# sbelharbi/sr-caco-2

Hardware: AMD Instinct MI355X
Metric: train patches/sec, SwinIR x8 64->512 1ch (higher is better)
Workload: dtype f32 (fp16x2 split-MFMA, f32 accumulate)

## Files before the change

### include/srhip.h

```cpp
#ifndef SRHIP_H
#define SRHIP_H
#ifdef __cplusplus
extern "C" {
#endif
#if defined(__GNUC__) || defined(__clang__)
#pragma GCC visibility push(default)
#endif

const char* srhip_last_error(void);
int srhip_abi_version(void);
int srhip_experiments_enabled(void);
int srhip_set_matmul_mode(int mode);
int srhip_get_matmul_mode(void);


int srhip_gemm_nt(const float* A, long lda, const float* W, long ldw, const float* bias, float* C,
                  long ldc, int M, int N, int K, int a_mode, const float* ln_stats, int epi,
                  const float* R, long ldr, const float* rowscale, int rows_per_scale, float alpha,
                  float* aux, long ldaux, void* stream);

int srhip_gemm_nt_batched(const float* A, long lda, long a_z0, long a_z1, const float* W, long ldw, long w_z0, long w_z1, float* C,
                          long ldc, long c_z0, long c_z1, int M, int N, int K, int zcount, int zdiv, void* stream);

int srhip_conv3x3_nhwc(const float* X, long ldx, const float* Wp, const float* bias, float* Y, long ldy,
// ... 13 lines not shown
int srhip_prep_table(const srhip_prep_entry* table_dev, int n, int total_blocks, void* stream);
int srhip_gemm_nt_bx3(const float* A, long lda, const void* Wb, const float* bias, float* C,
                      long ldc, int M, int N, int K, int a_mode, const float* ln_stats, int epi,
                      const float* R, long ldr, const float* rowscale, int rows_per_scale, float alpha,
                      float* aux, long ldaux, float* stats_out, void* stream);
int srhip_gemm_nt_bx3_lnbwd(const float* A, long lda, const void* Wb, float* out, long ldo, int M, int N, int K,
                            const float* x, long ldx, const float* stats, const float* res, long ldres,
                            void* stream);
int srhip_gemm_nt_f16x2(const float* A, long lda, const void* Wh, const float* bias, float* C,
                        long ldc, int M, int N, int K, int a_mode, const float* ln_stats, int epi,
                        const float* R, long ldr, const float* rowscale, int rows_per_scale, float alpha,
                        float* aux, long ldaux, float* stats_out, void* stream);
int srhip_gemm_nt_f16x2_lnbwd(const float* A, long lda, const void* Wh, float* out, long ldo, int M, int N, int K,
                              const float* x, long ldx, const float* stats, const float* res, long ldres,
                              void* stream);
int srhip_conv3x3_nhwc_f16x2(const float* X, long ldx, const void* Wh, const float* bias, float* Y, long ldy,
                             int B, int H, int W, int Cin, int Cout, int epi, const float* R, long ldr,
                             const float* rowscale, float alpha, void* stream);
int srhip_conv3x3_nhwc_split_ex(int wfmt, const float* X, long ldx, const void* Wp, const float* bias, float* Y, long ldy,
                                int B, int H, int W, int Cin, int Cout, int epi, const float* R, long ldr,
                                const float* rowscale, float alpha, const float* in_bn_coef, const float* slope,
                                void* stream);
int srhip_resblock64_fwd_f16x2(const float* x, long ldx, const void* W1h, const float* b1, const void* W2h, const float* b2,
                               float res_scale, float* a, long lda, float* out, long ldout, int B, int H, int W, void* stream);
int srhip_resblock64_bwd_f16x2(const float* g, long ldg, const void* W2Th, const void* W1Th, const float* a, long lda,
                               float res_scale, float* da, long ldda, float* dx, long lddx, int B, int H, int W, void* stream);

int srhip_conv3x3_nhwc_h16(const void* X, long ldx, const void* Wh, const float* bias, void* Y, long ldy, int B, int H, int W,
                           int Cin, int Cout, int epi, const void* R, long ldr, float alpha, int ps2, const float* in_bn_coef,
                           int center_only, void* stream);
// ... 207 lines not shown
int srhip_avgpool2d(const float* x, float* out, int B, int H, int W, int C, int k, void* stream);
int srhip_cpb_bias(const float* table, const long long* index, float* biasT, int heads, int N1, int N2, int entries, void* stream);
int srhip_cosine_window_attention(const float* q, long ldq, int qH, int qW, int qwh, int qww, const float* k, long ldk,
                                  const float* v, long ldv, int kH, int kW, int kwh, int kww, const float* logit_scale,
                                  const float* biasT, float* out, long ldo, int B, int heads, int d, int shift, void* stream);

int srhip_bias_expand_f16x2(const float* table, float* biasF, float* biasG, int heads, void* stream);
int srhip_window_attention_fwd_f16x2(const float* qkv, float* out, const float* biasF, int B, int H, int W, int C,
                                     int heads, int shift, void* stream);
long srhip_window_attention_bwd_f16x2_ws(int B, int H, int W, int heads);
int srhip_window_attention_bwd_f16x2(const float* qkv, const float* dout, float* dqkv, const float* biasF,
                                     const float* biasG, float* dbiasT, float* workspace, int B, int H, int W, int C,
                                     int heads, int shift, void* stream);
int srhip_window_attention_dbias_reduce_f16x2(const float* workspace, long ws_stride, int nblocks, float* dbiasT,
                                              long img_stride, int B, int H, int W, int heads, void* stream);

int srhip_bias_expand(const float* table, float* biasT, float* biasN, int heads, void* stream);
int srhip_bias_grad(const float* dbiasT, float* dtable, int heads, void* stream);
int srhip_bias_grad_batched(const float* dbiasT, long image_stride, float* const* dtables, int nblocks, int heads,
                            void* stream);
int srhip_window_attention_fwd(const float* qkv, float* out, const float* biasT, int B, int H, int W,
                               int C, int heads, int shift, void* stream);
long srhip_window_attention_bwd_ws(int B, int H, int W, int heads);
int srhip_window_attention_bwd(const float* qkv, const float* dout, float* dqkv, const float* biasT,
                               const float* biasN, float* dbiasT, float* workspace, int B, int H, int W,
                               int C, int heads, int shift, void* stream);

int srhip_conv3x3_cin1_fwd(const float* x, const float* w, const float* bias, float* y, long ldy, int B,
                           int H, int W, int Co, int flip, void* stream);
long srhip_conv3x3_cin1_wgrad_ws(int Co);
// ... 189 lines not shown
```

### sr-caco-2_amd/csrc/api.hip

```cpp
#include <stdarg.h>
#include "common.h"
#include "kernels.h"
#include "../../include/srhip.h"

static thread_local char g_err[512] = "";

int sr_fail(int code, const char* fmt, ...) {
  va_list ap;
  va_start(ap, fmt);
  vsnprintf(g_err, sizeof(g_err), fmt, ap);
  va_end(ap);
  return code;
}

extern "C" {

const char* srhip_last_error(void) { return g_err; }
int srhip_abi_version(void) { return 14; }
int srhip_experiments_enabled(void) {
#ifdef SRHIP_EXPERIMENTS
  return 1;
#else
  return 0;
#endif
// ... 93 lines not shown
                      const float* R, long ldr, const float* rowscale, int rows_per_scale, float alpha, float* aux,
                      long ldaux, float* stats_out, void* stream) {
  return gemm_nt_split(0, A, lda, Wb, bias, C, ldc, M, N, K, a_mode, ln_stats, epi, R, ldr, rowscale, rows_per_scale, alpha,
                       aux, ldaux, stats_out, stream);
}
int srhip_gemm_nt_f16x2(const float* A, long lda, const void* Wh, const float* bias, float* C,
                        long ldc, int M, int N, int K, int a_mode, const float* ln_stats, int epi,
                        const float* R, long ldr, const float* rowscale, int rows_per_scale, float alpha, float* aux,
                        long ldaux, float* stats_out, void* stream) {
  return gemm_nt_split(1, A, lda, Wh, bias, C, ldc, M, N, K, a_mode, ln_stats, epi, R, ldr, rowscale, rows_per_scale, alpha,
                       aux, ldaux, stats_out, stream);
}

static int gemm_nt_split_lnbwd(int wfmt, const float* A, long lda, const void* Wb, float* out, long ldo, int M, int N, int K,
                            const float* x, long ldx, const float* stats, const float* res, long ldres,
                            void* stream) {
  NtArgs p;
  memset(&p, 0, sizeof(p));
  p.A = A; p.lda = lda; p.Wb = (const unsigned short*)Wb; p.C = out; p.ldc = ldo;
  p.M = M; p.N = N; p.K = K; p.R = x; p.ldr = ldx; p.R2 = res; p.ldr2 = ldres; p.ep_stats = stats;
  p.alpha = 1.f;
  p.wfmt = wfmt;
  SR_REQUIRE(!wfmt || N % 180 == 0 || N > 128, "gemm_nt_f16x2_lnbwd: N = %d does not run on 192-column tiles", N);
  return sr_gemm_ntb_lnbwd(p, (hipStream_t)stream);
}
int srhip_gemm_nt_bx3_lnbwd(const float* A, long lda, const void* Wb, float* out, long ldo, int M, int N, int K,
                            const float* x, long ldx, const float* stats, const float* res, long ldres,
                            void* stream) {
  return gemm_nt_split_lnbwd(0, A, lda, Wb, out, ldo, M, N, K, x, ldx, stats, res, ldres, stream);
}
int srhip_gemm_nt_f16x2_lnbwd(const float* A, long lda, const void* Wh, float* out, long ldo, int M, int N, int K,
                              const float* x, long ldx, const float* stats, const float* res, long ldres,
                              void* stream) {
  return gemm_nt_split_lnbwd(1, A, lda, Wh, out, ldo, M, N, K, x, ldx, stats, res, ldres, stream);
}

int srhip_mlp_fwd_f16x2(const float* x, long ldx, const float* stats, const void* W1h, const float* b1,
                        const void* W2h, const float* b2, float* h, long ldh, float* out, long ldo, int M, int C,
                        int hidden, const float* rowscale, int rows_per_scale, float* stats_out, void* stream) {
  SR_REQUIRE(x && stats && W1h && b1 && W2h && out, "mlp_fwd_f16x2: null operand");
  SR_REQUIRE(!rowscale || rows_per_scale > 0, "mlp_fwd_f16x2: rows_per_scale must be > 0");
  MlpF16Args p;
  memset(&p, 0, sizeof(p));
  p.X = x; p.ldx = ldx; p.ln_stats = stats;
  p.W1 = (const unsigned short*)W1h; p.N1 = hidden; p.K1 = C; p.Kp1 = sr_kp(C);
  p.W2 = (const unsigned short*)W2h; p.N2 = C; p.K2 = hidden; p.Kp2 = sr_kp(hidden);
  p.b1 = b1; p.b2 = b2; p.H = h; p.ldh = h ? ldh : 4; p.out = out; p.ldo = ldo; p.R = x; p.ldr = ldx;
  p.rowscale = rowscale; p.rows_per_scale = rows_per_scale; p.stats_out = stats_out;
  p.M = M; p.C = C; p.hid = hidden;
// ... 373 lines not shown
```

### sr-caco-2_amd/csrc/kernels.h

```cpp
#pragma once
#include <hip/hip_runtime.h>

struct NtArgs {
  const float* A; long lda;
  const float* W; long ldw; long wtap;
  float* C; long ldc;
  int M, N, K;
  int n_tile;
  int xcd_order;
  const float* bias;
  int a_mode;
  const float* ln_stats;
  int epi;
  const float* slope;
  const float* pro_coef;
  const float* R; long ldr;
  float* aux; long ldaux;
  const float* R2; long ldr2; const float* ep_stats;
  int wide_epi;
  float* stats_out;
  const float* rowscale; int rows_per_scale; float alpha;
  int batch, H, Wd, tiles_x, tiles_y;
  int dbg;
  int stagger;
  const unsigned short* Wb; int Kp;
  int amp;
  int ps;
  int k_rot;
  int wfmt;
  int zcount, zdiv;
  long zA[2], zW[2], zC[2];
};

// ... 132 lines not shown
```

### sr-caco-2_amd/csrc/nt_epi.h

```cpp
#pragma once
#include "common.h"
#include "kernels.h"

__device__ __forceinline__ float half_reduce16(float (&a)[16], int lane) {
#pragma unroll
  for (int n = 8, m = 16; n >= 1; n >>= 1, m >>= 1) {
    const bool up = lane & m;
#pragma unroll
    for (int i = 0; i < n; ++i) {
      const float s = up ? a[i] : a[i + n], k = up ? a[i + n] : a[i];
      a[i] = k + __shfl_xor(s, m, 64);
    }
  }
  return a[0] + __shfl_xor(a[0], 1, 64);
}
__device__ __forceinline__ int half_reduce16_row(int lane) {
  return ((lane >> 4) & 1) * 8 + ((lane >> 3) & 1) * 4 + ((lane >> 2) & 1) * 2 + ((lane >> 1) & 1);
}

template <int WN>
__device__ __forceinline__ void nt_row_stats(const NtArgs& p, f32x16 (&acc)[1][WN], int lane, int wm, int wn,
                                             int m0, int nvalid, float* red) {
  const int r = lane & 31;
  const float inv = 1.0f / (float)p.N;
// ... 229 lines not shown
  }
  const float t1 = half_reduce16(a1, lane), t2 = half_reduce16(a2, lane);
  const int qs = half_reduce16_row(lane);
  __syncthreads();
  if (!(lane & 1)) *(float2*)(red + ((wn * 64) + wm * 32 + mfma_row(qs, lane)) * 2) = float2{t1, t2};
  float rres[WN][16];
#pragma unroll
  for (int j = 0; j < WN; ++j) {
    const int col = min((wn * WN + j) * 32 + r, nvalid - 1);
#pragma unroll
    for (int q = 0; q < 16; ++q) {
      const int g = min(rbase + mfma_row(q, lane), p.M - 1);
      rres[j][q] = p.R2 ? p.R2[(long)g * p.ldr2 + col] : 0.f;
    }
  }
  __syncthreads();
  const float inv = 1.0f / (float)p.N;
#pragma unroll
  for (int q = 0; q < 16; ++q) {
    const int lr = wm * 32 + mfma_row(q, lane);
    const float2 p0 = *(const float2*)(red + lr * 2), p1 = *(const float2*)(red + (64 + lr) * 2);
    const float m1 = (p0.x + p1.x) * inv, m2 = (p0.y + p1.y) * inv;
    const bool rok = rbase + mfma_row(q, lane) < p.M;
#pragma unroll
    for (int j = 0; j < WN; ++j) {
      const int col = (wn * WN + j) * 32 + r;
      if (rok && col < nvalid)
        p.C[(long)(rbase + mfma_row(q, lane)) * p.ldc + col] =
            rres[j][q] + rs[q] * (acc[0][j][q] - m1 - xh[j][q] * m2);
    }
  }
}

template <int WN, bool STATS>
__device__ __forceinline__ void nt_epilogue_wide_impl(const NtArgs& p, f32x16 (&acc)[1][WN], int lane, int wave,
                                                 int wm, int wn, int n0, int nvalid, int m0, float* lds) {
  constexpr int P = 32 * WN + 8;
  constexpr int F4 = 8 * WN;
  constexpr int NIT = 32 * F4 / 64;
  const int r = lane & 31;
  float* tile = lds + wave * (32 * P);
  __syncthreads();
#pragma unroll
  for (int j = 0; j < WN; ++j) {
// ... 112 lines not shown
```

### sr-caco-2_amd/csrc/wattn2.hip

```cpp
#include "common.h"
#include "kernels.h"
#include "wattn2_dev.h"

namespace {

template <int D>
__global__ void __launch_bounds__(256, 3) k_wattn2_fwd(const float* __restrict__ qkv, float* __restrict__ out,
                                                      const float* __restrict__ biasF, long total, int H, int W,
                                                      int C, int heads, int shift, float scale) {
  const int lane = threadIdx.x & 63, wv = threadIdx.x >> 6;
  const long gid = sr_xcd_block(blockIdx.x, gridDim.x) * 4L + wv;
  if (gid >= total) return;
  const W2Geom geo = w2_decode(gid, heads, W / 8, H / 8, shift);
  w2_fwd_body<D>(qkv, out, biasF, geo, H, W, C, shift, scale, lane);
}

template <int D>
__device__ __forceinline__ void w2_gather_cols(const float* __restrict__ base, long pitch, const W2Geom& geo, int H, int W,
                                               int shift, int c, int g, u32x4 (&hi)[2][2], u32x4 (&lo)[2][2],
                                               float (&rinv)[2]) {
  float raw[2][2][8];
#pragma unroll
  for (int JJ = 0; JJ < 2; ++JJ)
#pragma unroll
// ... 27 lines not shown
__device__ __forceinline__ void w2_pack_pair(const f32x4& t0, const f32x4& t1, float sc, u32x4& hi, u32x4& lo) {
  unsigned h[4], l[4];
  split2_pair(t0[0] * sc, t0[1] * sc, h[0], l[0]);
  split2_pair(t0[2] * sc, t0[3] * sc, h[1], l[1]);
  split2_pair(t1[0] * sc, t1[1] * sc, h[2], l[2]);
  split2_pair(t1[2] * sc, t1[3] * sc, h[3], l[3]);
  hi = u32x4{h[0], h[1], h[2], h[3]};
  lo = u32x4{l[0], l[1], l[2], l[3]};
}
__device__ __forceinline__ f32x4 mfma3(const u32x4& ah, const u32x4& al, const u32x4& bh, const u32x4& bl, f32x4 acc) {
  acc = mfma16h(ah, bl, acc);
  acc = mfma16h(al, bh, acc);
  return mfma16h(ah, bh, acc);
}

constexpr int W2_DS = 4096;
constexpr int W3_PL = 64 * 64;
constexpr int W3_IMG = 2 * W3_PL;
constexpr int W3_WPB = 4;
constexpr int W3_LDS = 4 * W3_IMG + (W2_DS + 256 + 4 * 64 + 2 * 64) * 4;

typedef short w3_s16x4 __attribute__((__vector_size__(4 * sizeof(short))));
template <int CTRL>
__device__ __forceinline__ float w3_dpp(float v) {
  return __builtin_bit_cast(float, __builtin_amdgcn_update_dpp(0, __builtin_bit_cast(int, v), CTRL, 0xf, 0xf, true));
}
__device__ __forceinline__ int w3_slot(int row, int u) { return (row * 4 + (u ^ ((row >> 2) & 3))) * 16; }
__device__ __forceinline__ void w3_rows(const unsigned char* img, int T, int c, int g, u32x4& hi, u32x4& lo) {
  const unsigned char* p = img + w3_slot(16 * T + c, g);
  hi = *(const u32x4*)p;
// ... 17 lines not shown
  lo = w3_cols1(img + W3_PL, JJ, jd, c, g);
}
#ifndef W3_OCC
#define W3_OCC 3
#endif
#ifdef SRHIP_EXPERIMENTS
__device__ long long* g_w3_dbg = nullptr;
__device__ int g_w3_mode = 0;
#define W3_MODE(B) (g_w3_mode & (B))
#define SR_TS(K) \
  if (g_w3_dbg && lane == 0) g_w3_dbg[(((long)blockIdx.x * 4 + wv) * W3_WPB + wi) * 8 + (K)] = (long long)wall_clock64();
#else
#define SR_TS(K)
#define W3_MODE(B) 0
#endif
template <int D>
__global__ void __launch_bounds__(256, W3_OCC) k_wattn3_bwd(const float* __restrict__ qkv, const float* __restrict__ dout,
                                                      float* __restrict__ dqkv, const float* __restrict__ biasF,
                                                      float* __restrict__ part,
                                                      int nwin, int H, int W, int C, int heads, int shift, float scale) {
  extern __shared__ __attribute__((aligned(16))) unsigned char w3s[];
  unsigned char* const imQ = w3s;
  unsigned char* const imK = w3s + W3_IMG;
  unsigned char* const imV = w3s + 2 * W3_IMG;
  unsigned char* const imG = w3s + 3 * W3_IMG;
  float* const dsl = (float*)(w3s + 4 * W3_IMG);
  float* const tab = dsl + W2_DS;
  float* const rs = tab + 256;
  float* const lse = rs + 256;
  float* const dlt = lse + 64;
  const int tid = threadIdx.x, lane = tid & 63, c = lane & 15, g = lane >> 4;
  const int wv = __builtin_amdgcn_readfirstlane(tid >> 6);
  const int lb = sr_xcd_block(blockIdx.x, gridDim.x);
  const int head = lb % heads, wg = lb / heads;
// ... 221 lines not shown
          OK[jd] = mfma3(th, tl, dh, dlo, OK[jd]);
        }
      }
      float* op = dqb + (long)w2_token(geo, 16 * J + c, H, W, shift) * C3 + 4 * g;
      if (!W3_MODE(2))
#pragma unroll
      for (int jd = 0; jd < 2; ++jd) {
        w3_store<D>(op + C + 16 * jd, 16 * jd + 4 * g, OK[jd], dri);
        w3_store<D>(op + 2 * C + 16 * jd, 16 * jd + 4 * g, OV[jd], pri);
      }
    }
    SR_TS(5)
    sr_lds_barrier();
    SR_TS(6)
  }
  if (part) {
    float* dst = part + ((long)wg * heads + head) * W2_DS;
#pragma unroll
    for (int J = 0; J < 4; ++J) {
      const int o = w2_img_index(wv, J, lane);
      *(f32x4*)(dst + o) = *(const f32x4*)(dsl + o);
    }
  }
}

__global__ void __launch_bounds__(256) k_dbias2_reduce(const float* __restrict__ part, int nparts, int heads,
                                                       float* __restrict__ dimg, long part_stride, long img_stride) {
  __shared__ double sm[4][64][4];
  const int ln = threadIdx.x & 63, pg = threadIdx.x >> 6;
  const int hd = blockIdx.x >> 4, a = (blockIdx.x >> 3) & 1, b = (blockIdx.x >> 2) & 1, qh = blockIdx.x & 3;
  part += (long)blockIdx.y * part_stride;
  dimg += (long)blockIdx.y * img_stride;
  const int key = mfma_row(4 * qh, ln) + 32 * a, query = (ln & 31) + 32 * b;
  const int mine = w2_img_index(query >> 4, key >> 4, 16 * ((key >> 2) & 3) + (query & 15));
  const float* p = part + (long)hd * W2_DS + mine;
  const long ps = (long)heads * W2_DS;
  double s0 = 0.0, s1 = 0.0, s2 = 0.0, s3 = 0.0;
  int i = pg;
// ... 80 lines not shown
}

int srhip_window_attention_bwd_f16x2(const float* qkv, const float* dout, float* dqkv, const float* biasF,
                                     const float* biasG, float* dbiasT, float* workspace, int B, int H, int W, int C,
                                     int heads, int shift, void* stream) {
  if (int rc = w2_check(B, H, W, C, heads, shift)) return rc;
  SR_REQUIRE(!dbiasT || workspace, "window_attention_bwd_f16x2: workspace required for the bias gradient");
  const int D = C / heads;
  const int nwin = B * (H / 8) * (W / 8), nparts = sr_cdiv(nwin, 4);
  const float scale = 1.0f / sqrtf((float)D);
  hipStream_t st = (hipStream_t)stream;
  dim3 grid(nparts * heads), blk(256);
  float* part = workspace;
#define SR_WA(D_)                                                                                                       \
  if (D == D_)                                                                                                          \
    hipLaunchKernelGGL((k_wattn3_bwd<D_>), grid, blk, W3_LDS, st, qkv, dout, dqkv, biasF, part, nwin, H, W, C,        \
                       heads, shift, scale);
  SR_WA(30) SR_WA(10) SR_WA(16) SR_WA(32)
#undef SR_WA
  if (dbiasT)
    hipLaunchKernelGGL(k_dbias2_reduce, dim3(heads * 16), dim3(256), 0, st, part, nparts, heads, dbiasT, 0L, 0L);
  SR_LAUNCH_CHECK("window_attention_bwd_f16x2");
  return 0;
}

int srhip_window_attention_dbias_reduce_f16x2(const float* workspace, long ws_stride, int nblocks, float* dbiasT,
                                              long img_stride, int B, int H, int W, int heads, void* stream) {
  SR_REQUIRE(workspace && dbiasT && nblocks > 0 && nblocks <= 65535, "window_attention_dbias_reduce_f16x2: bad arguments");
  const int nparts = sr_cdiv(B * (H / 8) * (W / 8), 4);
  hipLaunchKernelGGL(k_dbias2_reduce, dim3(heads * 16, nblocks), dim3(256), 0, (hipStream_t)stream,
                     workspace, nparts, heads, dbiasT, ws_stride, img_stride);
  SR_LAUNCH_CHECK("window_attention_dbias_reduce_f16x2");
  return 0;
}

}
```

### sr-caco-2_amd/srhip/ops.py

```python
import ctypes

import torch

from . import probe
from ._lib import call, lib, struct, SrhipError


def _chk(*ts):
    for t in ts:
        if t is None:
            continue
        if not t.is_cuda:
            raise SrhipError("srhip ops need CUDA/HIP tensors (no CPU fallback exists)")
        if t.dtype not in (torch.float32, torch.float64, torch.int32):
            raise SrhipError(f"unsupported dtype {t.dtype}")


def _p(t):
    return None if t is None else t.data_ptr()


def _st():
    return torch.cuda.current_stream().cuda_stream

# ... 228 lines not shown


def gemm_nt_batched(A, a_z, W, w_z, C, c_z, M, N, K, zcount, zdiv):
    _chk(A, W, C)
    assert A.stride(-1) == 1 and W.stride(-1) == 1 and C.stride(-1) == 1
    args = (A.data_ptr(), A.stride(-2), a_z[0], a_z[1], W.data_ptr(), W.stride(-2), w_z[0], w_z[1],
            C.data_ptr(), C.stride(-2), c_z[0], c_z[1], M, N, K, zcount, zdiv, _st())
    if probe.on("gemm_batched"):
        with probe.timed(("gemm_batched", M, N, K, zcount), 2.0 * M * N * K * zcount, 4.0 * zcount * (M * K + N * K + M * N)):
            call("srhip_gemm_nt_batched", *args)
    else:
        call("srhip_gemm_nt_batched", *args)
    return C


def gemm_nt_lnbwd(A, W, x, stats, res, out):
    assert isinstance(W, Bx3)
    _chk(A, x, stats, res, out)
    M, K = A.shape
    assert W.K == K and x.shape == (M, W.rows) and out.shape == (M, W.rows)
    args = (_p(A), A.stride(0), _p(W.planes), _p(out), out.stride(0), M, W.rows, K,
            _p(x), x.stride(0), _p(stats), _p(res), 0 if res is None else res.stride(0), _st())
    name = "srhip_gemm_nt_f16x2_lnbwd" if W.fmt == 1 else "srhip_gemm_nt_bx3_lnbwd"
    if probe.on("gemm_nt"):
        with probe.timed(("gemm_nt", M, W.rows, K), 2.0 * M * W.rows * K, 4.0 * (M * K + W.rows * K + 3 * M * W.rows)):
            call(name, *args)
    else:
        call(name, *args)
    return out


def l2norm_rows_(x, k=1.0, eps=5e-5):
    _chk(x)
    assert x.dim() == 2 and x.stride(1) == 1
    call("srhip_l2norm_rows", _p(x), x.stride(0), x.shape[0], x.shape[1], float(eps), float(k), _st())
    return x


# ... 1042 lines not shown
def window_attention_bwd_f16(qkv, dout, dqkv, biasF, biasG, dbiasT, B, H, W, C, heads, shift, parts=None):
    _chk(qkv, dout, dqkv, biasF, biasG, dbiasT, parts)
    if parts is not None:
        ws, dbiasT = parts, None
    else:
        ws = SCRATCH.get("wattn2_ws", lib.srhip_window_attention_bwd_f16x2_ws(B, H, W, heads), device=qkv.device)
    args = (_p(qkv), _p(dout), _p(dqkv), _p(biasF), _p(biasG), _p(dbiasT), _p(ws), B, H, W, C, heads, shift, _st())
    if probe.on("wattn"):
        T = B * H * W
        with probe.timed(("wattn", "bwd", T, C), 10.0 * T * 64 * C, 4.0 * T * 7 * C):
            call("srhip_window_attention_bwd_f16x2", *args)
        return
    call("srhip_window_attention_bwd_f16x2", *args)


def window_attention_fwd_f16(qkv, out, biasF, B, H, W, C, heads, shift):
    _chk(qkv, out, biasF)
    args = (_p(qkv), _p(out), _p(biasF), B, H, W, C, heads, shift, _st())
    if probe.on("wattn"):
        T = B * H * W
        with probe.timed(("wattn", "fwd", T, C), 4.0 * T * 64 * C, 4.0 * T * 4 * C):
            call("srhip_window_attention_fwd_f16x2", *args)
        return
    call("srhip_window_attention_fwd_f16x2", *args)


def window_attention_fwd(qkv, out, biasT, B, H, W, C, heads, shift):
    _chk(qkv, out, biasT)
    if probe.on("wattn"):
        T = B * H * W
# ... 924 lines not shown
```

### sr-caco-2_amd/srhip/swinir_engine.py

```python
import os

import torch

from . import ops
from .engine import Engine


def net_dev(net):
    return net.conv_first.weight.device


class SwinIREngine(Engine):
    train_graph_default = True

    def __init__(self, net):
        super().__init__(net)
        self.C = net.embed_dim
        self.hid = int(net.embed_dim * net.mlp_ratio)
        self.scale = net.upscale
        self.ci = net.in_chans
        self.blocks = list(net.swin_blocks())
        self.direct = net.upsampler == "pixelshuffledirect"
        self.nearest = net.upsampler == "nearest_conv"
        self.stages = 0 if (self.direct or self.nearest) else int(round(__import__("math").log2(net.upscale)))
# ... 380 lines not shown
            for i in range(self.stages):
                c = buf(f"upc{i}", B, h, w, 4 * nf)
                ops.conv3x3(u, ws[f"up{i}.wp"], net.upsample[2 * i].bias.data, 4 * nf, out=c)
                u = buf(f"upu{i}", B, 2 * h, 2 * w, nf)
                ops.pixel_shuffle(c, 2, nhwc_out=True, out=u)
                h, w = 2 * h, 2 * w
                ups.append(u)
            conv_last(u, h, w)
            if save:
                sv["ups"] = ups
        if save:
            sv.update(t_last=t, st_n=st_n, tn=tn, f=f)
            self.saved = sv
        return y

    def _bias_table_grads(self, layer, pre, dparts, dbT_all, bi0, j_lo, j_hi, lheads, B, H, W, G):
        if j_hi <= j_lo:
            return
        tabs = [G(pre + f"residual_group.blocks.{j}.attn.relative_position_bias_table") for j in range(j_lo, j_hi)]
        same = len(lheads) == 1
        if dparts is not None:
            ops.wattn_dbias_reduce_f16(dparts[j_lo:j_hi], dbT_all, bi0 + j_lo, B, H, W, next(iter(lheads)))
        for j0 in range(0, j_hi - j_lo, 8):
            if same:
                ops.bias_grad_batched(dbT_all, bi0 + j_lo + j0, tabs[j0:j0 + 8])
            else:
                for j in range(j_lo + j0, min(j_hi, j_lo + j0 + 8)):
                    ops.bias_grad(dbT_all[bi0 + j, :layer.residual_group.blocks[j].num_heads], tabs[j - j_lo])

    def backward(self, dy, grads, need_dx=False, on_layer_done=None, grads_zeroed=False):
        sv = self.saved_for_backward()
        net, C, hid, D, ws = self.net, self.C, self.hid, self.derived, self.ws
        B, H, W, dp = sv["B"], sv["H"], sv["W"], sv["dp"]
        T = B * H * W
# ... 122 lines not shown
        ops.layernorm_bwd(dtn, sv["t_last"], sv["st_n"], dt, gamma=net.norm.weight.data,
                          dgamma=G("norm.weight"), dbeta=G("norm.bias"))
        def layer_bufs(par):
            sfx = f".p{par}" if side_on else ""
            return ([buf(f"g{i}{sfx}", T, C) for i in range(2 * nset + 1)], [buf(f"dh{i}{sfx}", T, hid) for i in range(nset)],
                    [buf(f"dqkv{i}{sfx}", T, 3 * C) for i in range(nset)], sfx)
        gbufs, dhs, dqkvs, sfx = layer_bufs(0)
        recompute_gh = (self.fuse_mlp_h and ws.use_bx3 and ops.F16X2 and os.environ.get("SRHIP_RECOMPUTE_GH", "0") == "1")
        saved_gate = all(blk_sv[7] is not None for blk_sv in sv["blocks"])
        no_gh = recompute_gh or saved_gate
        ghs = [None if no_gh else buf(f"gh{i}", T, hid) for i in range(nset)]
        ghs2 = [None if no_gh else buf(f"gh{i}.p1", T, hid) for i in range(nset)] if side_on else ghs
        dxh, da = buf("dxh", T, C), buf("da", T, C)
        nrot = len(gbufs)
        bi = len(self.blocks)
        dbT_all = buf("dbiasT_all", len(self.blocks), max(b.num_heads for b in self.blocks), 64, 64)
        for li in reversed(range(len(net.layers))):
            layer = net.layers[li]
            t_in, t_blocks, rc = sv["layers"][li]
            pre = f"layers.{li}."
            if side_on:
                gbufs, dhs, dqkvs, sfx = layer_bufs(li & 1)
                if len(side_done) >= 2:
                    main_stream.wait_event(side_done[-2])
            ghs_l = ghs2 if (side_on and (li & 1)) else ghs
            gi = 0
            g = gbufs[gi]
            conv_done = resi_conv_bwd(f"l{li}", pre + "conv.", dt.view(B, H, W, C), t_blocks.view(B, H, W, C), rc,
                                      g.view(B, H, W, C))
            nb = len(layer.residual_group.blocks)
            cuts = {}
            if li == 0 and on_layer_done is not None and len(net.layers) > 1 and defer:
                grp = self.layer0_bucket_groups()
                if grp is not None:
                    cuts[grp[0][0]] = len(net.layers) - 1
                    if grp[1]:
                        cuts[grp[1][0]] = len(net.layers)
            flushed_hi = nb
            pending = []
            front = None
            lheads = {blk.num_heads for blk in layer.residual_group.blocks}
            dparts = None
            if len(lheads) == 1 and ops.wattn_f16_ok(C, next(iter(lheads))):
                nbmax = max(len(l.residual_group.blocks) for l in net.layers)
                dparts = buf("dbias_parts" + (f".p{li & 1}" if side_on else ""), nbmax,
                             ops.wattn_dbias_ws(B, H, W, max(b.num_heads for b in self.blocks)))
                dparts = dparts[:nb, :ops.wattn_dbias_ws(B, H, W, next(iter(lheads)))]
            for j in reversed(range(nb)):
                bi -= 1
                dh, gh, dqkv = dhs[j % nset], ghs_l[j % nset], dqkvs[j % nset]
                blk = layer.residual_group.blocks[j]
                p = pre + f"residual_group.blocks.{j}."
                t, st1, qkv, a, x1, st2, h, gate, ghf = sv["blocks"][bi]
                heads = blk.num_heads
                s1 = None if dp is None else dp[2 * bi]
                s2 = None if dp is None else dp[2 * bi + 1]
                g1, gout = gbufs[(gi + 1) % nrot], gbufs[(gi + 2) % nrot]
                chained = self.fuse_mlp_h and self.chain_proj and getattr(ws[f"{bi}.wpT"], "fmt", 0) == 1
# ... 2 lines not shown
                        gh = ghf
                    ops.mlp_bwd_f16(g, ws[f"{bi}.w2T"], ws[f"{bi}.w1T"], h, dh, None if gate is not None else gh, x1, st2, g1,
                                    rowscale=s2, rows_per_scale=H * W,
                                    chain=(ws[f"{bi}.wpT"], da, s1) if chained else None, front=front, gate=gate)
                    front = None
                else:
                    ops.gemm_nt(g, ws[f"{bi}.w2T"], None, out=dh, epi=3, R=h, rowscale=s2,
                                rows_per_scale=H * W, aux=gh)
                    if ws.use_bx3:
                        ops.gemm_nt_lnbwd(dh, ws[f"{bi}.w1T"], x1, st2, g, g1)
                    else:
                        ops.gemm_nt(dh, ws[f"{bi}.w1T"], None, out=dxh)
                        ops.layernorm_bwd(dxh, x1, st2, g1, res=g)
                if not chained:
                    ops.gemm_nt(g1, ws[f"{bi}.wpT"], None, out=da, epi=2, rowscale=s1, rows_per_scale=H * W)
                dbT = dbT_all[bi, :heads]
                if ops.wattn_f16_ok(C, heads):
                    ops.window_attention_bwd_f16(qkv, da, dqkv, D.d[f"{bi}.biasF"], D.d[f"{bi}.biasG"], dbT, B, H,
                                                 W, C, heads, blk.shift_size,
                                                 parts=None if dparts is None else dparts[j])
                else:
                    ops.window_attention_bwd(qkv, da, dqkv, D.d[f"{bi}.biasT"], D.d[f"{bi}.biasN"], dbT, B, H,
                                             W, C, heads, blk.shift_size)
                if (ws.use_bx3 and self.fuse_mlp_h and self.front_qkv and j > 0
                        and getattr(ws[f"{bi}.wqT"], "fmt", 0) == 1 and not ops.lib.srhip_get_matmul_mode()):
                    front = (dqkv, ws[f"{bi}.wqT"], t, st1, g1)
                elif ws.use_bx3:
                    ops.gemm_nt_lnbwd(dqkv, ws[f"{bi}.wqT"], t, st1, g1, gout)
                else:
                    ops.gemm_nt(dqkv, ws[f"{bi}.wqT"], None, out=dxh)
                    ops.layernorm_bwd(dxh, t, st1, gout, res=g1)
                problems = [
                    dict(dY=dqkv, X=t, dW=G(p + "attn.qkv.weight"),
                         db=G(p + "attn.qkv.bias") if blk.attn.qkv.bias is not None else buf("dbq.unused", 3 * C), b_mode=1,
                         ln_stats=st1, ln=(blk.attn.qkv.weight.data, blk.norm1.weight.data,
                                           blk.norm1.bias.data, G(p + "norm1.weight"), G(p + "norm1.bias"))),
                    dict(dY=g, X=h if gh is None else gh, b_mode=2 if gh is None else 0, dW=G(p + "mlp.fc2.weight"),
                         db=G(p + "mlp.fc2.bias"), a_rowscale=s2, a_rowscale_rows=H * W),
                    dict(dY=dh, X=x1, dW=G(p + "mlp.fc1.weight"), db=G(p + "mlp.fc1.bias"), b_mode=1,
                         ln_stats=st2, ln=(blk.mlp.fc1.weight.data, blk.norm2.weight.data,
                                           blk.norm2.bias.data, G(p + "norm2.weight"), G(p + "norm2.bias"))),
                    dict(dY=g1, X=a, dW=G(p + "attn.proj.weight"), db=G(p + "attn.proj.bias"),
                         a_rowscale=s1, a_rowscale_rows=H * W),
                ]
                if defer:
                    pending += problems
                else:
                    ops.linear_wgrad_grouped(problems)
                gi = (gi + 2) % nrot
                g = gout
                if j in cuts:
                    def cut_end(pending=pending, flushed_hi=flushed_hi, j=j, bi=bi):
                        ops.linear_wgrad_grouped(pending)
                        self._bias_table_grads(layer, pre, dparts, dbT_all, bi - j, j, flushed_hi, lheads, B, H, W, G)
                        on_layer_done(cuts[j])
                    side(cut_end)
                    pending = []
                    flushed_hi = j
            def layer_end(pending=pending, layer=layer, pre=pre, dparts=dparts, bi=bi, flushed_hi=flushed_hi, lheads=lheads, li=li,
                          cuts=cuts):
                if pending:
                    ops.linear_wgrad_grouped(pending)
                self._bias_table_grads(layer, pre, dparts, dbT_all, bi, 0, flushed_hi, lheads, B, H, W, G)
                if on_layer_done is not None and not cuts:
                    on_layer_done(len(net.layers) - 1 - li)
            side_done.append(side(layer_end))
            if conv_done is not None:
                main_stream.wait_event(conv_done)
            ops.axpby(dt, g, 1.0, 1.0)
        if side_on:
            main_stream.wait_stream(self.wstream)
        if net.ape:
            dpos = G("absolute_pos_embed").view(H * W, C)
            dpos.copy_(dt[:H * W])
            for b in range(1, B):
                ops.axpby(dpos, dt[b * H * W:(b + 1) * H * W], 1.0, 1.0)
        df0 = buf("df0", T, C)
        if net.patch_norm:
            ops.layernorm_bwd(dt, sv["f0"].view(T, C), sv["st_pe"], df0, res=df.view(T, C),
                              gamma=net.patch_embed.norm.weight.data, dgamma=G("patch_embed.norm.weight"),
                              dbeta=G("patch_embed.norm.bias"))
        else:
            df0.copy_(dt)
            ops.axpby(df0, df.view(T, C), 1.0, 1.0)
# ... 14 lines not shown
```

Baseline: 756.9.

## Bin relative-position bias grads in attention backward and fuse skip add into GEMM

The window-attention backward kernel can now reduce the 64x64 bias gradient straight into the 225 relative-position bins per head, writing them in double precision. A small batched reduce kernel then writes the bias-table gradients directly, replacing the full dbiasT buffer and the separate bias_grad scatter. Separately, the layer's final qkv LayerNorm-backward GEMM takes an extra addend and writes the skip-connection gradient straight into dt, which removes the per-layer axpby pass. The costs are more epilogue loads and fp64 accumulation work in the attention kernel, and the main stream now waits on the conv event before that GEMM rather than at the layer end.

Measured after the change: 753.9. No clear change (-0.4%).

```diff
diff --git a/include/srhip.h b/include/srhip.h
--- a/include/srhip.h
+++ b/include/srhip.h
@@ -51,6 +51,12 @@
 int srhip_gemm_nt_f16x2_lnbwd(const float* A, long lda, const void* Wh, float* out, long ldo, int M, int N, int K,
                               const float* x, long ldx, const float* stats, const float* res, long ldres,
                               void* stream);
+int srhip_gemm_nt_bx3_lnbwd_add(const float* A, long lda, const void* Wb, float* out, long ldo, int M, int N, int K,
+                                const float* x, long ldx, const float* stats, const float* res, long ldres,
+                                const float* add, long ldadd, void* stream);
+int srhip_gemm_nt_f16x2_lnbwd_add(const float* A, long lda, const void* Wh, float* out, long ldo, int M, int N, int K,
+                                  const float* x, long ldx, const float* stats, const float* res, long ldres,
+                                  const float* add, long ldadd, void* stream);
 int srhip_conv3x3_nhwc_f16x2(const float* X, long ldx, const void* Wh, const float* bias, float* Y, long ldy,
                              int B, int H, int W, int Cin, int Cout, int epi, const float* R, long ldr,
                              const float* rowscale, float alpha, void* stream);
@@ -288,6 +294,12 @@
                                      int heads, int shift, void* stream);
 int srhip_window_attention_dbias_reduce_f16x2(const float* workspace, long ws_stride, int nblocks, float* dbiasT,
                                               long img_stride, int B, int H, int W, int heads, void* stream);
+long srhip_window_attention_bwd_f16x2_tab_ws(int B, int H, int W, int heads);
+int srhip_window_attention_bwd_f16x2_tab(const float* qkv, const float* dout, float* dqkv, const float* biasF,
+                                         double* workspace, int B, int H, int W, int C, int heads, int shift,
+                                         void* stream);
+int srhip_window_attention_dtable_reduce_f16x2(const double* workspace, long ws_stride, float* const* dtables,
+                                               int nblocks, int B, int H, int W, int heads, void* stream);
 
 int srhip_bias_expand(const float* table, float* biasT, float* biasN, int heads, void* stream);
 int srhip_bias_grad(const float* dbiasT, float* dtable, int heads, void* stream);
diff --git a/sr-caco-2_amd/csrc/api.hip b/sr-caco-2_amd/csrc/api.hip
--- a/sr-caco-2_amd/csrc/api.hip
+++ b/sr-caco-2_amd/csrc/api.hip
@@ -131,11 +131,12 @@
 
 static int gemm_nt_split_lnbwd(int wfmt, const float* A, long lda, const void* Wb, float* out, long ldo, int M, int N, int K,
                             const float* x, long ldx, const float* stats, const float* res, long ldres,
-                            void* stream) {
+                            void* stream, const float* add = nullptr, long ldadd = 0) {
   NtArgs p;
   memset(&p, 0, sizeof(p));
   p.A = A; p.lda = lda; p.Wb = (const unsigned short*)Wb; p.C = out; p.ldc = ldo;
   p.M = M; p.N = N; p.K = K; p.R = x; p.ldr = ldx; p.R2 = res; p.ldr2 = ldres; p.ep_stats = stats;
+  p.R3 = add; p.ldr3 = ldadd;
   p.alpha = 1.f;
   p.wfmt = wfmt;
   SR_REQUIRE(!wfmt || N % 180 == 0 || N > 128, "gemm_nt_f16x2_lnbwd: N = %d does not run on 192-column tiles", N);
@@ -150,6 +151,18 @@
                               const float* x, long ldx, const float* stats, const float* res, long ldres,
                               void* stream) {
   return gemm_nt_split_lnbwd(1, A, lda, Wh, out, ldo, M, N, K, x, ldx, stats, res, ldres, stream);
+}
+int srhip_gemm_nt_bx3_lnbwd_add(const float* A, long lda, const void* Wb, float* out, long ldo, int M, int N, int K,
+                                const float* x, long ldx, const float* stats, const float* res, long ldres,
+                                const float* add, long ldadd, void* stream) {
+  SR_REQUIRE(add, "gemm_nt_bx3_lnbwd_add: the addend is required");
+  return gemm_nt_split_lnbwd(0, A, lda, Wb, out, ldo, M, N, K, x, ldx, stats, res, ldres, stream, add, ldadd);
+}
+int srhip_gemm_nt_f16x2_lnbwd_add(const float* A, long lda, const void* Wh, float* out, long ldo, int M, int N, int K,
+                                  const float* x, long ldx, const float* stats, const float* res, long ldres,
+                                  const float* add, long ldadd, void* stream) {
+  SR_REQUIRE(add, "gemm_nt_f16x2_lnbwd_add: the addend is required");
+  return gemm_nt_split_lnbwd(1, A, lda, Wh, out, ldo, M, N, K, x, ldx, stats, res, ldres, stream, add, ldadd);
 }
 
 int srhip_mlp_fwd_f16x2(const float* x, long ldx, const float* stats, const void* W1h, const float* b1,
diff --git a/sr-caco-2_amd/csrc/kernels.h b/sr-caco-2_amd/csrc/kernels.h
--- a/sr-caco-2_amd/csrc/kernels.h
+++ b/sr-caco-2_amd/csrc/kernels.h
@@ -17,6 +17,7 @@
   const float* R; long ldr;
   float* aux; long ldaux;
   const float* R2; long ldr2; const float* ep_stats;
+  const float* R3; long ldr3;
   int wide_epi;
   float* stats_out;
   const float* rowscale; int rows_per_scale; float alpha;
diff --git a/sr-caco-2_amd/csrc/nt_epi.h b/sr-caco-2_amd/csrc/nt_epi.h
--- a/sr-caco-2_amd/csrc/nt_epi.h
+++ b/sr-caco-2_amd/csrc/nt_epi.h
@@ -267,6 +267,16 @@
       rres[j][q] = p.R2 ? p.R2[(long)g * p.ldr2 + col] : 0.f;
     }
   }
+  float r3[WN][16];
+#pragma unroll
+  for (int j = 0; j < WN; ++j) {
+    const int col = min((wn * WN + j) * 32 + r, nvalid - 1);
+#pragma unroll
+    for (int q = 0; q < 16; ++q) {
+      const int g = min(rbase + mfma_row(q, lane), p.M - 1);
+      r3[j][q] = p.R3 ? p.R3[(long)g * p.ldr3 + col] : 0.f;
+    }
+  }
   __syncthreads();
   const float inv = 1.0f / (float)p.N;
 #pragma unroll
@@ -278,9 +288,8 @@
 #pragma unroll
     for (int j = 0; j < WN; ++j) {
       const int col = (wn * WN + j) * 32 + r;
-      if (rok && col < nvalid)
-        p.C[(long)(rbase + mfma_row(q, lane)) * p.ldc + col] =
-            rres[j][q] + rs[q] * (acc[0][j][q] - m1 - xh[j][q] * m2);
+      const float v = rres[j][q] + rs[q] * (acc[0][j][q] - m1 - xh[j][q] * m2);
+      if (rok && col < nvalid) p.C[(long)(rbase + mfma_row(q, lane)) * p.ldc + col] = p.R3 ? v + r3[j][q] : v;
     }
   }
 }
diff --git a/sr-caco-2_amd/csrc/wattn2.hip b/sr-caco-2_amd/csrc/wattn2.hip
--- a/sr-caco-2_amd/csrc/wattn2.hip
+++ b/sr-caco-2_amd/csrc/wattn2.hip
@@ -65,6 +65,7 @@
   return mfma16h(ah, bh, acc);
 }
 
+constexpr int W2_BINS = 225;
 constexpr int W2_DS = 4096;
 constexpr int W3_PL = 64 * 64;
 constexpr int W3_IMG = 2 * W3_PL;
@@ -112,10 +113,10 @@
 #define SR_TS(K)
 #define W3_MODE(B) 0
 #endif
-template <int D>
+template <int D, bool TAB = false>
 __global__ void __launch_bounds__(256, W3_OCC) k_wattn3_bwd(const float* __restrict__ qkv, const float* __restrict__ dout,
                                                       float* __restrict__ dqkv, const float* __restrict__ biasF,
-                                                      float* __restrict__ part,
+                                                      float* __restrict__ part, double* __restrict__ tpart,
                                                       int nwin, int H, int W, int C, int heads, int shift, float scale) {
   extern __shared__ __attribute__((aligned(16))) unsigned char w3s[];
   unsigned char* const imQ = w3s;
@@ -367,7 +368,7 @@
     sr_lds_barrier();
     SR_TS(6)
   }
-  if (part) {
+  if (!TAB && part) {
     float* dst = part + ((long)wg * heads + head) * W2_DS;
 #pragma unroll
     for (int J = 0; J < 4; ++J) {
@@ -375,6 +376,49 @@
       *(f32x4*)(dst + o) = *(const f32x4*)(dsl + o);
     }
   }
+  if (TAB && tid < W2_BINS) {
+    int bin = tid;
+    asm volatile("" : "+v"(bin));
+    const int dy = bin / 15 - 7, dx = bin % 15 - 7;
+    const int qy0 = max(dy, 0), qy1 = min(7, 7 + dy), qx0 = max(dx, 0), qx1 = min(7, 7 + dx);
+    double s = 0.0;
+#pragma unroll
+    for (int i = 0; i < 8; ++i) {
+      float v[8];
+#pragma unroll
+      for (int j = 0; j < 8; ++j) {
+        const int qy = min(qy0 + i, qy1), qx = min(qx0 + j, qx1);
+        const int query = 8 * qy + qx, key = 8 * (qy - dy) + (qx - dx);
+        v[j] = dsl[w2_img_index(query >> 4, key >> 4, 16 * ((key & 15) >> 2) + (query & 15)) + (key & 3)];
+      }
+#pragma unroll
+      for (int j = 0; j < 8; ++j) s += (qy0 + i <= qy1 && qx0 + j <= qx1) ? (double)v[j] : 0.0;
+    }
+    tpart[((long)wg * heads + head) * W2_BINS + bin] = s;
+  }
+}
+
+struct DtableBatch {
+  float* dtable[8];
+};
+__global__ void __launch_bounds__(64) k_dtable_reduce(const double* __restrict__ tpart, long ws_stride, int nparts,
+                                                       int heads, DtableBatch batch) {
+  const int i = blockIdx.x * blockDim.x + threadIdx.x;
+  if (i >= W2_BINS * heads) return;
+  const int bin = i / heads, hd = i - bin * heads;
+  const double* p = tpart + (long)blockIdx.y * ws_stride + (long)hd * W2_BINS + bin;
+  const long ps = (long)heads * W2_BINS;
+  double s = 0.0;
+  int n = 0;
+  for (; n + 32 <= nparts; n += 32) {
+    double v[32];
+#pragma unroll
+    for (int u = 0; u < 32; ++u) v[u] = p[(long)(n + u) * ps];
+#pragma unroll
+    for (int u = 0; u < 32; ++u) s += v[u];
+  }
+  for (; n < nparts; ++n) s += p[(long)n * ps];
+  batch.dtable[blockIdx.y][i] = (float)s;
 }
 
 __global__ void __launch_bounds__(256) k_dbias2_reduce(const float* __restrict__ part, int nparts, int heads,
@@ -485,8 +529,8 @@
   float* part = workspace;
 #define SR_WA(D_)                                                                                                       \
   if (D == D_)                                                                                                          \
-    hipLaunchKernelGGL((k_wattn3_bwd<D_>), grid, blk, W3_LDS, st, qkv, dout, dqkv, biasF, part, nwin, H, W, C,        \
-                       heads, shift, scale);
+    hipLaunchKernelGGL((k_wattn3_bwd<D_>), grid, blk, W3_LDS, st, qkv, dout, dqkv, biasF, part, (double*)nullptr, nwin, \
+                       H, W, C, heads, shift, scale);
   SR_WA(30) SR_WA(10) SR_WA(16) SR_WA(32)
 #undef SR_WA
   if (dbiasT)
@@ -505,4 +549,46 @@
   return 0;
 }
 
-}
+long srhip_window_attention_bwd_f16x2_tab_ws(int B, int H, int W, int heads) {
+  const int nwin = B * (H / 8) * (W / 8);
+  return (long)sr_cdiv(nwin, W3_WPB) * heads * W2_BINS;
+}
+
+int srhip_window_attention_bwd_f16x2_tab(const float* qkv, const float* dout, float* dqkv, const float* biasF,
+                                         double* workspace, int B, int H, int W, int C, int heads, int shift,
+                                         void* stream) {
+  if (int rc = w2_check(B, H, W, C, heads, shift)) return rc;
+  SR_REQUIRE(workspace && ((size_t)workspace & 7) == 0, "window_attention_bwd_f16x2_tab: an 8-byte aligned workspace is required");
+  const int D = C / heads;
+  const int nwin = B * (H / 8) * (W / 8), nparts = sr_cdiv(nwin, W3_WPB);
+  const float scale = 1.0f / sqrtf((float)D);
+  hipStream_t st = (hipStream_t)stream;
+  dim3 grid(nparts * heads), blk(256);
+#define SR_WA(D_)                                                                                                       \
+  if (D == D_)                                                                                                          \
+    hipLaunchKernelGGL((k_wattn3_bwd<D_, true>), grid, blk, W3_LDS, st, qkv, dout, dqkv, biasF, (float*)nullptr, workspace,  \
+                       nwin, H, W, C, heads, shift, scale);
+  SR_WA(30) SR_WA(10) SR_WA(16) SR_WA(32)
+#undef SR_WA
+  SR_LAUNCH_CHECK("window_attention_bwd_f16x2_tab");
+  return 0;
+}
+
+int srhip_window_attention_dtable_reduce_f16x2(const double* workspace, long ws_stride, float* const* dtables,
+                                               int nblocks, int B, int H, int W, int heads, void* stream) {
+  SR_REQUIRE(workspace && dtables && heads > 0, "window_attention_dtable_reduce_f16x2: null operand");
+  SR_REQUIRE(nblocks >= 1 && nblocks <= 8, "window_attention_dtable_reduce_f16x2: 1..8 blocks per launch (got %d)", nblocks);
+  DtableBatch b;
+  memset(&b, 0, sizeof(b));
+  for (int i = 0; i < nblocks; ++i) {
+    SR_REQUIRE(dtables[i] != nullptr, "window_attention_dtable_reduce_f16x2: table %d missing", i);
+    b.dtable[i] = dtables[i];
+  }
+  const int nparts = sr_cdiv(B * (H / 8) * (W / 8), W3_WPB);
+  hipLaunchKernelGGL(k_dtable_reduce, dim3(sr_cdiv(W2_BINS * heads, 64), nblocks), dim3(64), 0, (hipStream_t)stream,
+                     workspace, ws_stride, nparts, heads, b);
+  SR_LAUNCH_CHECK("window_attention_dtable_reduce_f16x2");
+  return 0;
+}
+
+}
diff --git a/sr-caco-2_amd/srhip/ops.py b/sr-caco-2_amd/srhip/ops.py
--- a/sr-caco-2_amd/srhip/ops.py
+++ b/sr-caco-2_amd/srhip/ops.py
@@ -266,14 +266,18 @@
     return C
 
 
-def gemm_nt_lnbwd(A, W, x, stats, res, out):
+def gemm_nt_lnbwd(A, W, x, stats, res, out, add=None):
     assert isinstance(W, Bx3)
-    _chk(A, x, stats, res, out)
+    _chk(A, x, stats, res, out, add)
     M, K = A.shape
     assert W.K == K and x.shape == (M, W.rows) and out.shape == (M, W.rows)
     args = (_p(A), A.stride(0), _p(W.planes), _p(out), out.stride(0), M, W.rows, K,
             _p(x), x.stride(0), _p(stats), _p(res), 0 if res is None else res.stride(0), _st())
     name = "srhip_gemm_nt_f16x2_lnbwd" if W.fmt == 1 else "srhip_gemm_nt_bx3_lnbwd"
+    if add is not None:
+        assert add.shape == (M, W.rows) and add.stride(1) == 1
+        args = args[:-1] + (_p(add), add.stride(0), _st())
+        name += "_add"
     if probe.on("gemm_nt"):
         with probe.timed(("gemm_nt", M, W.rows, K), 2.0 * M * W.rows * K, 4.0 * (M * K + W.rows * K + 3 * M * W.rows)):
             call(name, *args)
@@ -1346,6 +1350,33 @@
     call("srhip_window_attention_bwd_f16x2", *args)
 
 
+def wattn_dtable_ws(B, H, W, heads):
+    return lib.srhip_window_attention_bwd_f16x2_tab_ws(B, H, W, heads)
+
+
+def window_attention_bwd_f16_tab(qkv, dout, dqkv, biasF, tparts, B, H, W, C, heads, shift):
+    _chk(qkv, dout, dqkv, biasF, tparts)
+    assert tparts.dtype == torch.float64 and tparts.is_contiguous() and tparts.numel() >= wattn_dtable_ws(B, H, W, heads)
+    args = (_p(qkv), _p(dout), _p(dqkv), _p(biasF), _p(tparts), B, H, W, C, heads, shift, _st())
+    if probe.on("wattn"):
+        T = B * H * W
+        with probe.timed(("wattn", "bwd", T, C), 10.0 * T * 64 * C, 4.0 * T * 7 * C):
+            call("srhip_window_attention_bwd_f16x2_tab", *args)
+        return
+    call("srhip_window_attention_bwd_f16x2_tab", *args)
+
+
+def wattn_dtable_reduce_f16(tparts, dtables, B, H, W):
+    _chk(tparts, *dtables)
+    n, heads = len(dtables), dtables[0].shape[1]
+    assert tparts.dtype == torch.float64 and tparts.dim() == 2 and tparts.stride(1) == 1 and tparts.shape[0] == n
+    assert tparts.shape[1] >= wattn_dtable_ws(B, H, W, heads)
+    assert all(t.shape == (225, heads) and t.is_contiguous() and t.dtype == torch.float32 for t in dtables)
+    arr = (ctypes.c_void_p * n)(*[t.data_ptr() for t in dtables])
+    call("srhip_window_attention_dtable_reduce_f16x2", _p(tparts), tparts.stride(0), ctypes.addressof(arr), n,
+         B, H, W, heads, _st())
+
+
 def window_attention_fwd_f16(qkv, out, biasF, B, H, W, C, heads, shift):
     _chk(qkv, out, biasF)
     args = (_p(qkv), _p(out), _p(biasF), B, H, W, C, heads, shift, _st())
diff --git a/sr-caco-2_amd/srhip/swinir_engine.py b/sr-caco-2_amd/srhip/swinir_engine.py
--- a/sr-caco-2_amd/srhip/swinir_engine.py
+++ b/sr-caco-2_amd/srhip/swinir_engine.py
@@ -418,10 +418,14 @@
             self.saved = sv
         return y
 
-    def _bias_table_grads(self, layer, pre, dparts, dbT_all, bi0, j_lo, j_hi, lheads, B, H, W, G):
+    def _bias_table_grads(self, layer, pre, dparts, dbT_all, bi0, j_lo, j_hi, lheads, B, H, W, G, tparts=None):
         if j_hi <= j_lo:
             return
         tabs = [G(pre + f"residual_group.blocks.{j}.attn.relative_position_bias_table") for j in range(j_lo, j_hi)]
+        if tparts is not None:
+            for j0 in range(0, j_hi - j_lo, 8):
+                ops.wattn_dtable_reduce_f16(tparts[j_lo + j0:min(j_hi, j_lo + j0 + 8)], tabs[j0:j0 + 8], B, H, W)
+            return
         same = len(lheads) == 1
         if dparts is not None:
             ops.wattn_dbias_reduce_f16(dparts[j_lo:j_hi], dbT_all, bi0 + j_lo, B, H, W, next(iter(lheads)))
@@ -574,7 +578,14 @@
         dxh, da = buf("dxh", T, C), buf("da", T, C)
         nrot = len(gbufs)
         bi = len(self.blocks)
-        dbT_all = buf("dbiasT_all", len(self.blocks), max(b.num_heads for b in self.blocks), 64, 64)
+        tab_bins = os.environ.get("SRHIP_DTABLE_BINS", "1") != "0"
+
+        def table_form(layer):
+            lh = {blk.num_heads for blk in layer.residual_group.blocks}
+            return tab_bins and len(lh) == 1 and ops.wattn_f16_ok(C, next(iter(lh)))
+        dbT_all = (None if all(table_form(l) for l in net.layers)
+                   else buf("dbiasT_all", len(self.blocks), max(b.num_heads for b in self.blocks), 64, 64))
+        skip_in_gemm = ws.use_bx3 and os.environ.get("SRHIP_SKIP_IN_GEMM", "1") != "0"
         for li in reversed(range(len(net.layers))):
             layer = net.layers[li]
             t_in, t_blocks, rc = sv["layers"][li]
@@ -600,8 +611,14 @@
             pending = []
             front = None
             lheads = {blk.num_heads for blk in layer.residual_group.blocks}
-            dparts = None
-            if len(lheads) == 1 and ops.wattn_f16_ok(C, next(iter(lheads))):
+            dparts = tparts = None
+            if table_form(layer):
+                nbmax = max(len(l.residual_group.blocks) for l in net.layers)
+                tparts = bufs.get("g.dtable_parts" + (f".p{li & 1}" if side_on else ""), nbmax,
+                                  ops.wattn_dtable_ws(B, H, W, max(b.num_heads for b in self.blocks)), device=dev,
+                                  dtype=torch.float64)
+                tparts = tparts[:nb, :ops.wattn_dtable_ws(B, H, W, next(iter(lheads)))]
+            elif len(lheads) == 1 and ops.wattn_f16_ok(C, next(iter(lheads))):
                 nbmax = max(len(l.residual_group.blocks) for l in net.layers)
                 dparts = buf("dbias_parts" + (f".p{li & 1}" if side_on else ""), nbmax,
                              ops.wattn_dbias_ws(B, H, W, max(b.num_heads for b in self.blocks)))
@@ -634,8 +651,11 @@
                         ops.layernorm_bwd(dxh, x1, st2, g1, res=g)
                 if not chained:
                     ops.gemm_nt(g1, ws[f"{bi}.wpT"], None, out=da, epi=2, rowscale=s1, rows_per_scale=H * W)
-                dbT = dbT_all[bi, :heads]
-                if ops.wattn_f16_ok(C, heads):
+                dbT = None if tparts is not None else dbT_all[bi, :heads]
+                if tparts is not None:
+                    ops.window_attention_bwd_f16_tab(qkv, da, dqkv, D.d[f"{bi}.biasF"], tparts[j], B, H, W, C, heads,
+                                                     blk.shift_size)
+                elif ops.wattn_f16_ok(C, heads):
                     ops.window_attention_bwd_f16(qkv, da, dqkv, D.d[f"{bi}.biasF"], D.d[f"{bi}.biasG"], dbT, B, H,
                                                  W, C, heads, blk.shift_size,
                                                  parts=None if dparts is None else dparts[j])
@@ -645,6 +665,10 @@
                 if (ws.use_bx3 and self.fuse_mlp_h and self.front_qkv and j > 0
                         and getattr(ws[f"{bi}.wqT"], "fmt", 0) == 1 and not ops.lib.srhip_get_matmul_mode()):
                     front = (dqkv, ws[f"{bi}.wqT"], t, st1, g1)
+                elif ws.use_bx3 and j == 0 and skip_in_gemm:
+                    if conv_done is not None:
+                        main_stream.wait_event(conv_done)
+                    ops.gemm_nt_lnbwd(dqkv, ws[f"{bi}.wqT"], t, st1, g1, dt, add=dt)
                 elif ws.use_bx3:
                     ops.gemm_nt_lnbwd(dqkv, ws[f"{bi}.wqT"], t, st1, g1, gout)
                 else:
@@ -672,22 +696,24 @@
                 if j in cuts:
                     def cut_end(pending=pending, flushed_hi=flushed_hi, j=j, bi=bi):
                         ops.linear_wgrad_grouped(pending)
-                        self._bias_table_grads(layer, pre, dparts, dbT_all, bi - j, j, flushed_hi, lheads, B, H, W, G)
+                        self._bias_table_grads(layer, pre, dparts, dbT_all, bi - j, j, flushed_hi, lheads, B, H, W, G,
+                                               tparts=tparts)
                         on_layer_done(cuts[j])
                     side(cut_end)
                     pending = []
                     flushed_hi = j
             def layer_end(pending=pending, layer=layer, pre=pre, dparts=dparts, bi=bi, flushed_hi=flushed_hi, lheads=lheads, li=li,
-                          cuts=cuts):
+                          cuts=cuts, tparts=tparts):
                 if pending:
                     ops.linear_wgrad_grouped(pending)
-                self._bias_table_grads(layer, pre, dparts, dbT_all, bi, 0, flushed_hi, lheads, B, H, W, G)
+                self._bias_table_grads(layer, pre, dparts, dbT_all, bi, 0, flushed_hi, lheads, B, H, W, G, tparts=tparts)
                 if on_layer_done is not None and not cuts:
                     on_layer_done(len(net.layers) - 1 - li)
             side_done.append(side(layer_end))
-            if conv_done is not None:
-                main_stream.wait_event(conv_done)
-            ops.axpby(dt, g, 1.0, 1.0)
+            if not skip_in_gemm:
+                if conv_done is not None:
+                    main_stream.wait_event(conv_done)
+                ops.axpby(dt, g, 1.0, 1.0)
         if side_on:
             main_stream.wait_stream(self.wstream)
         if net.ape:
```
